# resibots/limbo

Measured on NVIDIA H100. Metric: GP fit+query/s at N=16384,D=6 (fit = K-build+Cholesky+alpha, query = 10k UCB candidates+argmax, fp64), higher is better.
Workload: dtype f64

## Files before the change

limbo_b200/csrc/gemm.cuh:

```cuda
#pragma once
#include "common.cuh"

namespace lbg {

constexpr int BM = 128;
constexpr int STAGES = 3;
constexpr int MMA_K = 4;

template <int BN_, int WN_, int BK_>
struct Cfg {
    static constexpr int BN = BN_, WN = WN_, BK = BK_;
    static constexpr int THREADS = 128 * WN;
    static constexpr int NT = BN / (8 * WN);
    static constexpr int PITCH_A_OC = BM + 4;
    static constexpr int PITCH_B_OC = BN + 4;
    static constexpr int PITCH_KC = BK + 4;
    static constexpr int A_STAGE = (BM * PITCH_KC > BK * PITCH_A_OC) ? BM * PITCH_KC : BK * PITCH_A_OC;
    static constexpr int B_STAGE = (BN * PITCH_KC > BK * PITCH_B_OC) ? BN * PITCH_KC : BK * PITCH_B_OC;
    static constexpr size_t PIPE_BYTES = (size_t)STAGES * (A_STAGE + B_STAGE) * sizeof(double);
    static constexpr int A_PIPE_DOUBLES = STAGES * A_STAGE;
    static_assert(BN % (8 * WN) == 0 && BK % MMA_K == 0, "tile shape");
    static_assert(PITCH_KC % 16 == 4 && PITCH_A_OC % 16 == 4 && PITCH_B_OC % 16 == 4, "conflict-free pitches");
};
using CfgWide = Cfg<128, 4, 32>;
using CfgDual = Cfg<64, 2, 16>;
using CfgStep = Cfg<64, 4, 32>;

template <typename C, bool KC, int NOUTER, int PITCH_OC>
struct TilePlan {
    static constexpr int CHUNKS = NOUTER * C::BK / 2;
    static constexpr int PER_THREAD = (CHUNKS + C::THREADS - 1) / C::THREADS;
    static constexpr int CPR = KC ? C::BK / 2 : NOUTER / 2;
    static constexpr int ROWS_PER_Q = C::THREADS / CPR;
    static constexpr int SSTEP = ROWS_PER_Q * (KC ? C::PITCH_KC : PITCH_OC);
    static_assert(C::THREADS % CPR == 0, "every chunk of a thread sits in the same column of the slab");
    int64_t goff, gstep;
    int soff;
    __device__ __forceinline__ void init(int64_t ld)
    {
        const int row = threadIdx.x / CPR, cc = threadIdx.x - row * CPR;
        goff = (int64_t)row * ld + 2 * cc;
        gstep = (int64_t)ROWS_PER_Q * ld;
        soff = row * (KC ? C::PITCH_KC : PITCH_OC) + 2 * cc;
    }
    __device__ __forceinline__ void issue(double* s, const double* __restrict__ g) const
    {
        s += soff;
        g += goff;
#pragma unroll
        for (int q = 0; q < PER_THREAD; ++q)
            if (CHUNKS % C::THREADS == 0 || (int)threadIdx.x + q * C::THREADS < CHUNKS) lb_cp_async16(s + q * SSTEP, g + q * gstep);
    }
};

template <typename C>
struct Acc {
    double v[2][C::NT][4];
    __device__ __forceinline__ void zero()
    {
#pragma unroll
        for (int a = 0; a < 2; ++a)
#pragma unroll
            for (int b = 0; b < C::NT; ++b)
#pragma unroll
                for (int c = 0; c < 4; ++c) v[a][b][c] = 0.0;
    }
};

template <typename C, bool NEG_A, typename FA, typename FB>
__device__ __forceinline__ void mma_kstep(Acc<C>& acc, FA fa, FB fb)
{
    double a[2][MMA_K / 2], b[C::NT][MMA_K / 4];
#pragma unroll
    for (int mt = 0; mt < 2; ++mt)
#pragma unroll
        for (int i = 0; i < MMA_K / 2; ++i) {
            a[mt][i] = fa(mt * 16 + 8 * (i & 1), 4 * (i >> 1));
            if (NEG_A) a[mt][i] = -a[mt][i];
        }
#pragma unroll
    for (int nt = 0; nt < C::NT; ++nt)
#pragma unroll
        for (int i = 0; i < MMA_K / 4; ++i) b[nt][i] = fb(nt * 8, 4 * i);
#pragma unroll
    for (int nt = 0; nt < C::NT; ++nt)
#pragma unroll
        for (int mt = 0; mt < 2; ++mt) lb_dmma_16x8<MMA_K>(acc.v[mt][nt], a[mt], b[nt]);
}

template <typename C, bool A_KC, bool B_KC, bool NEG_A>
__device__ __forceinline__ void compute_stage(Acc<C>& acc, const double* sA, const double* sB)
{
    const int lane = threadIdx.x & 31, warp = threadIdx.x >> 5;
    const int g = lane >> 2, t = lane & 3;
    const int wm = warp & 3, wn = warp >> 2;
    const int m_base = wm * 32 + g, n_base = wn * (C::BN / C::WN) + g;
#pragma unroll 2
    for (int k0 = 0; k0 < C::BK; k0 += MMA_K) {
        const int k = k0 + t;
        mma_kstep<C, NEG_A>(
            acc,
            [&](int dm, int dk) { return A_KC ? sA[(m_base + dm) * C::PITCH_KC + k + dk] : sA[(k + dk) * C::PITCH_A_OC + m_base + dm]; },
            [&](int dn, int dk) { return B_KC ? sB[(n_base + dn) * C::PITCH_KC + k + dk] : sB[(k + dk) * C::PITCH_B_OC + n_base + dn]; });
    }
}

template <typename C, bool A_KC, bool B_KC, bool NEG_A = false>
__device__ __forceinline__ void mainloop(Acc<C>& acc, const double* __restrict__ gA, int64_t lda,
    const double* __restrict__ gB, int64_t ldb, int K, double* smem)
{
    double* sA = smem;
    double* sB = smem + C::A_PIPE_DOUBLES;
    const int nk = K / C::BK;
    const int64_t stepA = A_KC ? C::BK : (int64_t)C::BK * lda;
    const int64_t stepB = B_KC ? C::BK : (int64_t)C::BK * ldb;
    TilePlan<C, A_KC, BM, C::PITCH_A_OC> pa;
    TilePlan<C, B_KC, C::BN, C::PITCH_B_OC> pb;
    pa.init(lda);
    pb.init(ldb);
#pragma unroll
    for (int s = 0; s < STAGES - 1; ++s) {
        if (s < nk) {
            pa.issue(sA + s * C::A_STAGE, gA + s * stepA);
            pb.issue(sB + s * C::B_STAGE, gB + s * stepB);
        }
        lb_cp_async_commit();
    }
    for (int kt = 0; kt < nk; ++kt) {
        lb_cp_async_wait<STAGES - 2>();
        __syncthreads();
        const int s = kt % STAGES;
        compute_stage<C, A_KC, B_KC, NEG_A>(acc, sA + s * C::A_STAGE, sB + s * C::B_STAGE);
        const int nx = kt + STAGES - 1;
        if (nx < nk) {
            const int sn = nx % STAGES;
            pa.issue(sA + sn * C::A_STAGE, gA + nx * stepA);
            pb.issue(sB + sn * C::B_STAGE, gB + nx * stepB);
        }
        lb_cp_async_commit();
    }
    lb_cp_async_wait<0>();
    __syncthreads();
}

template <typename C, typename F>
__device__ __forceinline__ void for_each_acc(Acc<C>& acc, F&& f)
{
    const int lane = threadIdx.x & 31, warp = threadIdx.x >> 5;
    const int g = lane >> 2, t = lane & 3;
    const int wm = warp & 3, wn = warp >> 2;
#pragma unroll
    for (int mt = 0; mt < 2; ++mt)
#pragma unroll
        for (int nt = 0; nt < C::NT; ++nt)
#pragma unroll
            for (int i = 0; i < 4; ++i) {
                int row = wm * 32 + mt * 16 + g + 8 * (i >> 1);
                int col = wn * (C::BN / C::WN) + nt * 8 + 2 * t + (i & 1);
                f(row, col, acc.v[mt][nt][i]);
            }
}

template <typename C>
__device__ __forceinline__ void load_acc(Acc<C>& acc, const double* __restrict__ Cg, int64_t ld)
{
    for_each_acc<C>(acc, [&](int r, int c, double& v) { v = __ldcs(Cg + r + (int64_t)c * ld); });
}
template <typename C>
__device__ __forceinline__ void store_acc(Acc<C>& acc, double* __restrict__ Cg, int64_t ld)
{
    for_each_acc<C>(acc, [&](int r, int c, double& v) { Cg[r + (int64_t)c * ld] = v; });
}

template <typename C>
__device__ __forceinline__ void mainloop_resB(Acc<C>& acc, const double* __restrict__ gA, int64_t lda,
    const double* sBres, double* smem_pipe)
{
    constexpr int PB = BM + 4;
    constexpr int nk = BM / C::BK;
    const int lane = threadIdx.x & 31, warp = threadIdx.x >> 5;
    const int g = lane >> 2, t = lane & 3;
    const int wm = warp & 3, wn = warp >> 2;
    const int m_base = wm * 32 + g, n_base = wn * (C::BN / C::WN) + g;
    TilePlan<C, false, BM, C::PITCH_A_OC> pa;
    pa.init(lda);
#pragma unroll
    for (int s = 0; s < STAGES - 1; ++s) {
        pa.issue(smem_pipe + s * C::A_STAGE, gA + (int64_t)s * C::BK * lda);
        lb_cp_async_commit();
    }
    for (int kt = 0; kt < nk; ++kt) {
        lb_cp_async_wait<STAGES - 2>();
        __syncthreads();
        const int nx = kt + STAGES - 1;
        if (nx < nk) pa.issue(smem_pipe + (nx % STAGES) * C::A_STAGE, gA + (int64_t)nx * C::BK * lda);
        lb_cp_async_commit();
        const double* sA = smem_pipe + (kt % STAGES) * C::A_STAGE;
#pragma unroll
        for (int k0 = 0; k0 < C::BK; k0 += MMA_K) {
            const int k = k0 + t;
            mma_kstep<C, false>(
                acc, [&](int dm, int dk) { return sA[(k + dk) * C::PITCH_A_OC + m_base + dm]; },
                [&](int dn, int dk) { return sBres[(n_base + dn) * PB + kt * C::BK + k + dk]; });
        }
    }
    lb_cp_async_wait<0>();
    __syncthreads();
}

}
```

limbo_b200/csrc/potrf.cu:

```cuda
#include "gemm.cuh"
#include <cstdlib>

namespace {

constexpr int PS = LB_TILE + 4;
constexpr int XP = 36;
constexpr int XB = 32 * XP;
constexpr size_t POTF2_SMEM = (size_t)(LB_TILE * PS + 10 * XB + LB_TILE) * sizeof(double);

__device__ __forceinline__ int blk(int ib, int jb) { return ib * (ib + 1) / 2 + jb; }

template <typename FA, typename FB>
__device__ __forceinline__ void warp_mma(double (&c)[4], int K, FA fa, FB fb)
{
    constexpr int KS = lbg::MMA_K;
    const int lane = threadIdx.x & 31, g = lane >> 2, t = lane & 3;
    for (int k0 = 0; k0 < K; k0 += KS) {
        double a[KS / 2], b[KS / 4];
#pragma unroll
        for (int i = 0; i < KS / 2; ++i) a[i] = fa(g + 8 * (i & 1), k0 + t + 4 * (i >> 1));
#pragma unroll
        for (int i = 0; i < KS / 4; ++i) b[i] = fb(k0 + t + 4 * i, g);
        lb_dmma_16x8<KS>(c, a, b);
    }
// ... 138 lines not shown
        }
        __syncthreads();
        const double* Xd = Xb + blk(ib, ib) * XB;
        for (int w = warp; w < 8 * ib; w += 8) {
            const int jb = w >> 3, mt = (w >> 2) & 1, nt = w & 3;
            double c[4] = {0.0, 0.0, 0.0, 0.0};
            warp_mma(c, 32, [&](int m, int kk) { return Xd[kk * XP + 16 * mt + m]; },
                [&](int kk, int n) { return S[(32 * ib + 8 * nt + n) * PS + 32 * jb + kk]; });
            double* Xo = Xb + blk(ib, jb) * XB;
#pragma unroll
            for (int e = 0; e < 4; ++e) Xo[(8 * nt + 2 * t + (e & 1)) * XP + 16 * mt + g + 8 * (e >> 1)] = -c[e];
        }
        __syncthreads();
    }
    LB_TICK();
    double* inv_out = invD + (int64_t)k * LB_TILE * LB_TILE;
    for (int idx = tid; idx < LB_TILE * (LB_TILE / 2); idx += 256) {
        const int c = idx >> 6, r = (idx & 63) * 2;
        if (c > r + 1) continue;
        if (do_factor) {
            double2 v = *reinterpret_cast<const double2*>(&S[c * PS + r]);
            if (c > r) v.x = 0.0;
            if (c > r + 1) v.y = 0.0;
            *reinterpret_cast<double2*>(Lkk + r + (int64_t)c * ld) = v;
        }
        double2 x = make_double2(0.0, 0.0);
        if (c <= r + 1) {
            const double* Xs_ = Xb + blk(r >> 5, c >> 5) * XB + (c & 31) * XP + (r & 31);
            x = *reinterpret_cast<const double2*>(Xs_);
            if (c > r) x.x = 0.0;
        }
        *reinterpret_cast<double2*>(inv_out + r + c * LB_TILE) = x;
    }
    __syncthreads();
    LB_TICK();
#undef LB_TICK
}

__global__ void __launch_bounds__(lbg::CfgWide::THREADS, 1)
trsm_panel_kernel(double* __restrict__ L, int64_t ld, int k, const double* __restrict__ invD)
{
    using C = lbg::CfgWide;
    extern __shared__ __align__(16) double smem[];
    const int i = k + 1 + blockIdx.x;
    double* A = L + (int64_t)i * LB_TILE + (int64_t)k * LB_TILE * ld;
    const double* B = invD + (int64_t)k * LB_TILE * LB_TILE;
    lbg::Acc<C> acc;
    acc.zero();
    lbg::mainloop<C, false, false>(acc, A, ld, B, LB_TILE, LB_TILE, smem);
    lbg::store_acc<C>(acc, A, ld);
}

template <typename C>
__global__ void __launch_bounds__(C::THREADS, (C::THREADS == 256) ? 2 : 1)
syrk_kernel(double* __restrict__ L, int64_t ld, int kb, int kd, int j0, int nc, int T)
{
    extern __shared__ __align__(16) double smem[];
    constexpr int SPLIT = LB_TILE / C::BN;
    int idx = blockIdx.x / SPLIT, c = 0;
    const int h = blockIdx.x - idx * SPLIT;
    while (c < nc && idx >= T - j0 - c) { idx -= T - j0 - c; ++c; }
    const int j = j0 + c, i = j + idx;
    const double* A = L + (int64_t)i * LB_TILE + (int64_t)kb * LB_TILE * ld;
    const double* B = L + (int64_t)j * LB_TILE + h * C::BN + (int64_t)kb * LB_TILE * ld;
    double* Cg = L + (int64_t)i * LB_TILE + ((int64_t)j * LB_TILE + h * C::BN) * ld;
    lbg::Acc<C> acc;
    lbg::load_acc<C>(acc, Cg, ld);
    lbg::mainloop<C, false, false, true>(acc, A, ld, B, ld, kd * LB_TILE, smem);
    lbg::store_acc<C>(acc, Cg, ld);
}

using SyrkCfg = lbg::CfgDual;
constexpr int SYRK_SPLIT = LB_TILE / SyrkCfg::BN;

LbOncePerDevice g_attr_once;
int set_attrs()
{
    if (!g_attr_once.need()) return LB_OK;
    LB_CUDA(cudaFuncSetAttribute(potf2_inv_kernel, cudaFuncAttributeMaxDynamicSharedMemorySize, (int)POTF2_SMEM));
    LB_CUDA(cudaFuncSetAttribute(trsm_panel_kernel, cudaFuncAttributeMaxDynamicSharedMemorySize, (int)lbg::CfgWide::PIPE_BYTES));
    LB_CUDA(cudaFuncSetAttribute(syrk_kernel<SyrkCfg>, cudaFuncAttributeMaxDynamicSharedMemorySize, (int)SyrkCfg::PIPE_BYTES));
    LB_CUDA(cudaFuncSetAttribute(syrk_kernel<lbg::CfgWide>, cudaFuncAttributeMaxDynamicSharedMemorySize, (int)lbg::CfgWide::PIPE_BYTES));
    return LB_OK;
}

}

int lb_debug_potf2_clocks(lb_gp* h, int k, long long* out_host, int n)
{
    int rc = set_attrs();
    if (rc) return rc;
    long long* d = nullptr;
    LB_CUDA(cudaMalloc(&d, sizeof(long long) * 16));
    LB_CUDA(cudaMemset(d, 0, sizeof(long long) * 16));
    potf2_inv_kernel<<<1, 256, POTF2_SMEM, h->stream>>>(h->dL, h->Np, k, h->dInvD, h->dInfo, 1, d);
    LB_CUDA(cudaStreamSynchronize(h->stream));
    LB_CUDA(cudaMemcpy(out_host, d, sizeof(long long) * (n < 16 ? n : 16), cudaMemcpyDeviceToHost));
    cudaFree(d);
    return LB_OK;
}

int lb_launch_potf2_block(lb_gp* h, int k, int do_factor)
{
    int rc = set_attrs();
    if (rc) return rc;
    potf2_inv_kernel<<<1, 256, POTF2_SMEM, h->stream>>>(h->dL, h->Np, k, h->dInvD, h->dInfo, do_factor);
    h->launches++;
    LB_CUDA(cudaGetLastError());
    return LB_OK;
}

static inline int syrk_tiles(int T, int j0, int nc)
{
    int n = 0;
    for (int c = 0; c < nc; ++c) n += T - j0 - c;
    return n;
}

static int launch_pair_panel(lb_gp* h, cudaStream_t side, int k, int T, int64_t ld)
{
    {
        LbProfScope ps(h, side, LB_PC_POTF2);
        potf2_inv_kernel<<<1, 256, POTF2_SMEM, side>>>(h->dL, ld, k, h->dInvD, h->dInfo, 1);
    }
    h->launches++;
    if (k + 1 < T) {
        {
            LbProfScope ps(h, side, LB_PC_TRSM_PANEL);
            trsm_panel_kernel<<<T - k - 1, lbg::CfgWide::THREADS, lbg::CfgWide::PIPE_BYTES, side>>>(h->dL, ld, k, h->dInvD);
        }
        {
            LbProfScope ps(h, side, LB_PC_SYRK_COL);
            syrk_kernel<SyrkCfg><<<(T - k - 1) * SYRK_SPLIT, SyrkCfg::THREADS, SyrkCfg::PIPE_BYTES, side>>>(h->dL, ld, k, 1, k + 1, 1, T);
        }
        {
            LbProfScope ps(h, side, LB_PC_POTF2);
            potf2_inv_kernel<<<1, 256, POTF2_SMEM, side>>>(h->dL, ld, k + 1, h->dInvD, h->dInfo, 1);
        }
        h->launches += 3;
        if (k + 2 < T) {
            LbProfScope ps(h, side, LB_PC_TRSM_PANEL);
            trsm_panel_kernel<<<T - k - 2, lbg::CfgWide::THREADS, lbg::CfgWide::PIPE_BYTES, side>>>(h->dL, ld, k + 1, h->dInvD);
            h->launches++;
        }
    }
    LB_CUDA(cudaGetLastError());
    return LB_OK;
}

static int launch_potrf_quads(lb_gp* h)
{
    const int T = (int)(h->Np / LB_TILE);
    const int64_t ld = h->Np;
    cudaStream_t main = h->stream, side = h->side ? h->side : h->stream;
    LB_CUDA(cudaMemsetAsync(h->dInfo, 0, 2 * sizeof(int), main));
    if (side != main) {
        LB_CUDA(cudaEventRecord(h->ev[0], main));
        LB_CUDA(cudaStreamWaitEvent(side, h->ev[0], 0));
    }
    int rc, q = 0;
    for (int k = 0; k < T; k += 4, ++q) {
        if ((rc = launch_pair_panel(h, side, k, T, ld))) return rc;
        if (k + 2 < T) {
            const int nc2 = (T - (k + 2) < 2) ? (T - (k + 2)) : 2;
            {
                LbProfScope ps(h, side, LB_PC_SYRK_COL);
                syrk_kernel<SyrkCfg><<<syrk_tiles(T, k + 2, nc2) * SYRK_SPLIT, SyrkCfg::THREADS, SyrkCfg::PIPE_BYTES, side>>>(h->dL, ld, k, 2, k + 2, nc2, T);
            }
            h->launches++;
            if ((rc = launch_pair_panel(h, side, k + 2, T, ld))) return rc;
        }
        if (k + 4 >= T) break;
        if (side != main) {
            LB_CUDA(cudaEventRecord(h->ev[1 + (q & 1)], side));
            LB_CUDA(cudaStreamWaitEvent(main, h->ev[1 + (q & 1)], 0));
        }
        const int j0 = k + 4;
        const int nca = (T - j0 < 4) ? (T - j0) : 4;
        static int wide = -1;
        if (wide < 0) { const char* e = getenv("LB_SYRK_WIDE"); wide = (e && atoi(e) != 0) ? 1 : 0; }
        {
            LbProfScope ps(h, main, LB_PC_SYRK);
            syrk_kernel<SyrkCfg><<<syrk_tiles(T, j0, nca) * SYRK_SPLIT, SyrkCfg::THREADS, SyrkCfg::PIPE_BYTES, main>>>(h->dL, ld, k, 4, j0, nca, T);
        }
        h->launches++;
        if (side != main) {
            LB_CUDA(cudaEventRecord(h->ev[3 + (q & 1)], main));
            LB_CUDA(cudaStreamWaitEvent(side, h->ev[3 + (q & 1)], 0));
        }
        const int ncb = T - j0 - nca;
        if (ncb > 0) {
            LbProfScope ps(h, main, LB_PC_SYRK);
            if (wide)
                syrk_kernel<lbg::CfgWide><<<syrk_tiles(T, j0 + nca, ncb), lbg::CfgWide::THREADS, lbg::CfgWide::PIPE_BYTES, main>>>(h->dL, ld, k, 4, j0 + nca,
                    ncb, T);
            else
                syrk_kernel<SyrkCfg><<<syrk_tiles(T, j0 + nca, ncb) * SYRK_SPLIT, SyrkCfg::THREADS, SyrkCfg::PIPE_BYTES, main>>>(h->dL, ld, k, 4, j0 + nca, ncb, T);
            h->launches++;
        }
    }
    if (side != main) {
        LB_CUDA(cudaEventRecord(h->ev[5], side));
        LB_CUDA(cudaStreamWaitEvent(main, h->ev[5], 0));
    }
    LB_CUDA(cudaGetLastError());
    return LB_OK;
}

int lb_launch_potrf(lb_gp* h)
{
    int rc = set_attrs();
    if (rc) return rc;
    static int quad = -1;
    if (quad < 0) { const char* e = getenv("LB_POTRF_QUAD"); quad = (e && atoi(e) == 0) ? 0 : 1; }
    if (quad) return launch_potrf_quads(h);
    const int T = (int)(h->Np / LB_TILE);
    const int64_t ld = h->Np;
    cudaStream_t main = h->stream, side = h->side ? h->side : h->stream;
    static int split_on = -1;
    if (split_on < 0) { const char* e = getenv("LB_POTRF_SPLIT"); split_on = (e && atoi(e) != 0) ? 1 : 0; }
    cudaStream_t second = main;
    if (split_on && T >= 24 && side != main) {
        if (!h->aux && cudaStreamCreateWithFlags(&h->aux, cudaStreamNonBlocking) != cudaSuccess) h->aux = nullptr;
        if (h->aux) second = h->aux;
    }
    const int cstar = (second != main) ? (((int)(0.38 * T)) & ~1) : T;
    LB_CUDA(cudaMemsetAsync(h->dInfo, 0, 2 * sizeof(int), main));
    if (side != main) {
        LB_CUDA(cudaEventRecord(h->ev[0], main));
        LB_CUDA(cudaStreamWaitEvent(side, h->ev[0], 0));
        if (second != main) LB_CUDA(cudaStreamWaitEvent(second, h->ev[0], 0));
    }
    int p = 0;
    for (int k = 0; k < T; k += 2, ++p) {
        const bool pair = (k + 1 < T);
        {
            LbProfScope ps(h, side, LB_PC_POTF2);
            potf2_inv_kernel<<<1, 256, POTF2_SMEM, side>>>(h->dL, ld, k, h->dInvD, h->dInfo, 1);
        }
        h->launches++;
        if (pair) {
            {
                LbProfScope ps(h, side, LB_PC_TRSM_PANEL);
                trsm_panel_kernel<<<T - k - 1, lbg::CfgWide::THREADS, lbg::CfgWide::PIPE_BYTES, side>>>(h->dL, ld, k, h->dInvD);
            }
            {
                LbProfScope ps(h, side, LB_PC_SYRK_COL);
                syrk_kernel<SyrkCfg><<<(T - k - 1) * SYRK_SPLIT, SyrkCfg::THREADS, SyrkCfg::PIPE_BYTES, side>>>(h->dL, ld, k, 1, k + 1, 1, T);
            }
            {
// ... 45 lines not shown
            if (ncb > 0) {
                LbProfScope ps(h, sa, LB_PC_SYRK);
                syrk_kernel<SyrkCfg><<<syrk_tiles(T, jb, ncb) * SYRK_SPLIT, SyrkCfg::THREADS, SyrkCfg::PIPE_BYTES, sa>>>(h->dL, ld, k, 2, jb, ncb, T);
                h->launches++;
            }
        }
    }
    if (side != main) {
        LB_CUDA(cudaEventRecord(h->ev[5], side));
        LB_CUDA(cudaStreamWaitEvent(main, h->ev[5], 0));
    }
    if (second != main) {
        LB_CUDA(cudaEventRecord(h->ev[6], second));
        LB_CUDA(cudaStreamWaitEvent(main, h->ev[6], 0));
    }
    LB_CUDA(cudaGetLastError());
    return LB_OK;
}

namespace {

__device__ __forceinline__ int dchol_global_block(int l, int rank, int G) { return 2 * (G * (l >> 1) + rank) + (l & 1); }

__global__ void __launch_bounds__(256)
dchol_build_kernel(const double* __restrict__ Xs, int64_t xs_ld, int64_t N, int64_t Nd, KernParams kp, int rank, int G, int64_t ncols_local,
    double* __restrict__ dLoc)
{
    const int64_t i = (int64_t)blockIdx.y * 256 + threadIdx.x;
    const int64_t c = blockIdx.x;
    if (i >= Nd || c >= ncols_local) return;
    const int64_t j = (int64_t)dchol_global_block((int)(c / LB_TILE), rank, G) * LB_TILE + (c % LB_TILE);
    double v;
    if (i >= N || j >= N) v = (i == j) ? 1.0 : 0.0;
    else {
        double z = 0.0;
        for (int d = 0; d < kp.D; ++d) {
            const double q = Xs[(int64_t)d * xs_ld + i] - Xs[(int64_t)d * xs_ld + j];
            z = fma(q, q, z);
        }
        v = lb_kernel_from_z(kp.id, z, kp) + ((i == j) ? kp.noise + 1e-8 : 0.0);
    }
    dLoc[i + c * Nd] = v;
}

__global__ void __launch_bounds__(256)
dchol_pack_kernel(const double* __restrict__ cols, int64_t ld, int64_t row0, double* __restrict__ panel, int64_t ldp)
{
    const int64_t r = (int64_t)blockIdx.x * 256 + threadIdx.x;
    const int c = blockIdx.y;
    if (r < ldp) panel[r + c * ldp] = cols[row0 + r + c * ld];
}

template <typename C>
__global__ void __launch_bounds__(C::THREADS, (C::THREADS == 256) ? 2 : 1)
dchol_update_kernel(double* __restrict__ Lloc, int64_t ld, const double* __restrict__ P, int64_t ldp, int kpair, int l0, int l1, int rank,
    int G, int T)
{
    extern __shared__ __align__(16) double smem[];
    constexpr int SPLIT = LB_TILE / C::BN;
    int idx = blockIdx.x / SPLIT;
    const int h = blockIdx.x - idx * SPLIT;
    int l = l0;
    for (; l < l1; ++l) {
        const int nt = T - dchol_global_block(l, rank, G);
        if (idx < nt) break;
        idx -= nt;
    }
    if (l >= l1) return;
    const int j = dchol_global_block(l, rank, G), i = j + idx;
    const int b0 = kpair + 2;
    const double* A = P + (int64_t)(i - b0) * LB_TILE;
    const double* B = P + (int64_t)(j - b0) * LB_TILE + h * C::BN;
    double* Cg = Lloc + (int64_t)i * LB_TILE + ((int64_t)l * LB_TILE + h * C::BN) * ld;
    lbg::Acc<C> acc;
    lbg::load_acc<C>(acc, Cg, ld);
    lbg::mainloop<C, false, false, true>(acc, A, ldp, B, ldp, 2 * LB_TILE, smem);
    lbg::store_acc<C>(acc, Cg, ld);
}

__global__ void __launch_bounds__(256)
dchol_finish_kernel(double* __restrict__ Lloc, int64_t ld, int64_t N, int rank, int G, int64_t ncols_local, double* __restrict__ part)
{
    __shared__ double red[8];
    double s = 0.0;
    for (int64_t c = blockIdx.x; c < ncols_local; c += gridDim.x) {
        const int64_t j = (int64_t)dchol_global_block((int)(c / LB_TILE), rank, G) * LB_TILE + (c % LB_TILE);
        double* col = Lloc + c * ld;
        for (int64_t i = threadIdx.x; i < j && i < ld; i += 256) col[i] = 0.0;
        if (threadIdx.x == 0 && j < N) s += log(col[j]);
    }
    s = lb_warp_sum(s);
    if ((threadIdx.x & 31) == 0) red[threadIdx.x >> 5] = s;
    __syncthreads();
    if (threadIdx.x == 0) {
        double t = 0.0;
        for (int w = 0; w < 8; ++w) t += red[w];
        part[blockIdx.x] = t;
    }
}
__global__ void dchol_sum_kernel(const double* __restrict__ part, int n, double* __restrict__ out)
{
    double s = 0.0;
    for (int i = 0; i < n; ++i) s += part[i];
    *out = s;
}

LbOncePerDevice g_dchol_once;
// ... 81 lines not shown
```

limbo_b200/csrc/query.cu:

```cuda
#include "gemm.cuh"
#include <cfloat>
#include <cstdlib>

namespace {

constexpr int DCH = 16;

__global__ void __launch_bounds__(256, 2)
kstar_kernel(const double* __restrict__ Xs, int64_t Np, int64_t N, const double* __restrict__ Qs, int64_t Mp,
    int64_t M, double* __restrict__ V, KernParams kp)
{
    __shared__ __align__(128) double sxi[DCH][LB_TILE];
    __shared__ __align__(128) double sxj[DCH][LB_TILE];
    __shared__ __align__(8) uint64_t bar;
    const int tid = threadIdx.x, lane = tid & 31, warp = tid >> 5;
    const int li = lane & 7, lj = lane >> 3;
    const int D = kp.D;
    const int64_t i0 = (int64_t)blockIdx.x * LB_TILE, j0 = (int64_t)blockIdx.y * LB_TILE;
    const int r0 = warp * 16 + 2 * li;
    if (tid == 0) {
        lb_mbar_init(&bar, 1);
        lb_fence_barrier_init();
    }
    __syncthreads();
// ... 590 lines not shown
        __syncthreads();
        if (tid < ncols && c0 + tid < M) {
            double res = kp.sf2 - sNrm[tid];
            res = (res <= DBL_EPSILON) ? 0.0 : res;
            s2_out[c0 + tid] = res + kp.noise;
            for (int p = 0; p < P; ++p) mu_out[(c0 + tid) * P + p] = sMu[p * SLAB + tid];
        }
        __syncthreads();
    }
}

__global__ void __launch_bounds__(THREADS, 1)
query_slab_kernel(const double* __restrict__ L, int64_t ld, const double* __restrict__ invD, const double* __restrict__ Xs,
    int64_t N, const double* __restrict__ Qs, int64_t Mp, int64_t M, const double* __restrict__ alpha, int P, KernParams kp,
    double* __restrict__ Vscratch, int nslabs, int64_t ntiles_total, double* __restrict__ mu_out, double* __restrict__ s2_out)
{
    extern __shared__ __align__(16) double sm[];
    double* V = Vscratch + (int64_t)blockIdx.x * ld * SLAB;
    for (int s = blockIdx.x; s < nslabs; s += gridDim.x) {
        const int64_t t0 = ntiles_total * s / nslabs, t1 = ntiles_total * (s + 1) / nslabs;
        const int ntc = (int)(t1 - t0);
        if (ntc == 9) slab_body<9>(sm, L, ld, invD, Xs, N, Qs, Mp, M, alpha, P, kp, V, t0, ntc, mu_out, s2_out);
        else if (ntc == 8) slab_body<8>(sm, L, ld, invD, Xs, N, Qs, Mp, M, alpha, P, kp, V, t0, ntc, mu_out, s2_out);
        else slab_body<0>(sm, L, ld, invD, Xs, N, Qs, Mp, M, alpha, P, kp, V, t0, ntc, mu_out, s2_out);
    }
}

struct PointArg { double x[LB_MAX_D]; };

__global__ void __launch_bounds__(THREADS, 1)
query_point_kernel(const double* __restrict__ L, int64_t ld, const double* __restrict__ invD, const double* __restrict__ Xs, int64_t N,
    const __grid_constant__ PointArg q, double* __restrict__ Qs, const double* __restrict__ alpha, int P, const __grid_constant__ KernParams kp,
    double* __restrict__ Vscratch, double* __restrict__ out)
{
    extern __shared__ __align__(16) double sm[];
    for (int idx = threadIdx.x; idx < kp.D * 8; idx += THREADS) {
        const int d = idx >> 3, c = idx & 7;
        Qs[d * LB_TILE + c] = (c == 0) ? lb_staged_coord(kp, d, [&](int r) { return q.x[r]; }) : 0.0;
    }
    __threadfence_block();
    __syncthreads();
    slab_body<0>(sm, L, ld, invD, Xs, N, Qs, LB_TILE, 1, alpha, P, kp, Vscratch, 0, 1, out, out + P);
}

LbOncePerDevice g_attr_once2;

}

namespace panel {

constexpr int SB = 16;

template <typename C, bool INV>
__global__ void __launch_bounds__(C::THREADS, (C::THREADS == 256) ? 2 : 1)
panel_update_kernel(const double* __restrict__ L, int64_t ld, const double* __restrict__ V, double* __restrict__ Tbuf, int64_t ldt, int s0,
    int nrows, int ct0, int inv_rank, int inv_G)
{
    extern __shared__ __align__(16) double smem[];
    const int i = blockIdx.x % nrows, ct = ct0 + blockIdx.x / nrows;
    int kb = 0;
    if (INV) {
        const int c = inv_rank + (ct * C::BN / LB_TILE) * inv_G;
        if (c >= s0 + nrows) return;
        kb = c / SB * SB;
    }
    const double* Vc = V + (int64_t)ct * C::BN * ld;
    lbg::Acc<C> acc;
    lbg::load_acc<C>(acc, Vc + (int64_t)(s0 + i) * LB_TILE, ld);
    if (s0 > kb)
        lbg::mainloop<C, false, true, true>(acc, L + (int64_t)(s0 + i) * LB_TILE + (int64_t)kb * LB_TILE * ld, ld, Vc + (int64_t)kb * LB_TILE, ld,
            (s0 - kb) * LB_TILE, smem);
    lbg::store_acc<C>(acc, Tbuf + (int64_t)i * LB_TILE + (int64_t)ct * C::BN * ldt, ldt);
}

template <typename C, bool INV>
__global__ void __launch_bounds__(C::THREADS, (C::THREADS == 256) ? 2 : 1)
panel_solve_kernel(const double* __restrict__ Linv, int64_t ld, const double* __restrict__ Tbuf, int64_t ldt, double* __restrict__ V, int s0,
    int nrows, double* __restrict__ normpart, int64_t Mp, int ct0, int inv_rank, int inv_G)
{
    extern __shared__ __align__(16) double smem[];
    const int i = nrows - 1 - (int)(blockIdx.x % nrows), ct = ct0 + blockIdx.x / nrows;
    int k0 = 0;
    if (INV) {
        const int c = inv_rank + (ct * C::BN / LB_TILE) * inv_G;
        if (c >= s0 + nrows) return;
        if (c > s0) k0 = c - s0;
        if (i < k0) return;
    }
    lbg::Acc<C> acc;
    acc.zero();
    lbg::mainloop<C, false, true>(acc, Linv + (int64_t)(s0 + i) * LB_TILE + (int64_t)(s0 + k0) * LB_TILE * ld, ld,
        Tbuf + (int64_t)k0 * LB_TILE + (int64_t)ct * C::BN * ldt, ldt, (i + 1 - k0) * LB_TILE, smem);
    lbg::store_acc<C>(acc, V + (int64_t)(s0 + i) * LB_TILE + (int64_t)ct * C::BN * ld, ld);
    if (INV) return;
    const int lane = threadIdx.x & 31, warp = threadIdx.x >> 5;
    const int g = lane >> 2, t = lane & 3;
    const int wm = warp & 3, wn = warp >> 2;
    double* sRed = smem;
#pragma unroll
    for (int nt = 0; nt < C::NT; ++nt)
#pragma unroll
        for (int e = 0; e < 2; ++e) {
            double sq = 0.0;
#pragma unroll
            for (int mt = 0; mt < 2; ++mt) {
                sq = fma(acc.v[mt][nt][e], acc.v[mt][nt][e], sq);
                sq = fma(acc.v[mt][nt][2 + e], acc.v[mt][nt][2 + e], sq);
            }
#pragma unroll
            for (int o = 4; o < 32; o <<= 1) sq += __shfl_xor_sync(0xffffffffu, sq, o);
            if (g == 0) sRed[wm * C::BN + wn * (C::BN / C::WN) + nt * 8 + 2 * t + e] = sq;
        }
    __syncthreads();
    if ((int)threadIdx.x < C::BN) {
        const double sum = ((sRed[threadIdx.x] + sRed[C::BN + threadIdx.x]) + sRed[2 * C::BN + threadIdx.x]) + sRed[3 * C::BN + threadIdx.x];
        normpart[(int64_t)(s0 + i) * Mp + (int64_t)ct * C::BN + threadIdx.x] = sum;
    }
}

__global__ void __launch_bounds__(256)
panel_finish_kernel(const double* __restrict__ normpart, int T, int64_t Mp, int64_t M, double kvv, double noise, double* __restrict__ s2)
{
    const int64_t c = blockIdx.x * (int64_t)256 + threadIdx.x;
    if (c >= M) return;
    double s = 0.0;
    for (int tt = 0; tt < T; ++tt) s += normpart[(int64_t)tt * Mp + c];
    double res = kvv - s;
    res = (res <= DBL_EPSILON) ? 0.0 : res;
    s2[c] = res + noise;
}

LbOncePerDevice g_once;

}

size_t lb_query_panel_scratch_doubles(const lb_gp* h, int64_t Mp)
{
    const int64_t T = h->Np / LB_TILE;
    return (size_t)(h->Np * Mp + (int64_t)panel::SB * LB_TILE * Mp + T * Mp);
}

int lb_launch_query_panel(lb_gp* h, cudaStream_t st, int64_t M, const double* dQs, int64_t Mp, double* dWork, double* dMu, double* dS2,
    long long* launches)
{
    using namespace panel;
    using CW = lbg::CfgWide;
    using CD = lbg::CfgDual;
    if (g_once.need()) {
        LB_CUDA(cudaFuncSetAttribute(panel_update_kernel<CW, false>, cudaFuncAttributeMaxDynamicSharedMemorySize, (int)CW::PIPE_BYTES));
        LB_CUDA(cudaFuncSetAttribute(panel_solve_kernel<CW, false>, cudaFuncAttributeMaxDynamicSharedMemorySize, (int)CW::PIPE_BYTES));
        LB_CUDA(cudaFuncSetAttribute(panel_update_kernel<CD, false>, cudaFuncAttributeMaxDynamicSharedMemorySize, (int)CD::PIPE_BYTES));
        LB_CUDA(cudaFuncSetAttribute(panel_solve_kernel<CD, false>, cudaFuncAttributeMaxDynamicSharedMemorySize, (int)CD::PIPE_BYTES));
    }
    const int T = (int)(h->Np / LB_TILE);
    const int64_t ld = h->Np, ldt = (int64_t)SB * LB_TILE;
    double* dV = dWork;
    double* dT = dV + ld * Mp;
    double* dNorm = dT + ldt * Mp;
    int rc = lb_launch_linv_levels(h, SB);
    if (rc) return rc;
    dim3 grid((unsigned)T, (unsigned)(Mp / LB_TILE));
    {
        LbProfScope ps(h, st, LB_PC_KSTAR);
        kstar_kernel<<<grid, 256, 0, st>>>(h->dXs, h->Np, h->N, dQs, Mp, M, dV, h->kp);
    }
    {
        LbProfScope ps(h, st, LB_PC_QREDUCE);
        mu_kernel<<<(unsigned)M, 256, 0, st>>>(dV, h->Np, h->dAlpha, h->P, dMu);
    }
    if (launches) *launches += 2;
    const int ctiles = (int)(Mp / LB_TILE);
    static int split_pct = -1, use_side = -1;
    if (split_pct < 0) {
        const char* e = getenv("LB_PANEL_SPLIT");
        split_pct = e ? atoi(e) : 100;
        if (split_pct < 1 || split_pct > 100) split_pct = 100;
        const char* e2 = getenv("LB_PANEL_SIDE");
        use_side = (e2 && atoi(e2) != 0) ? 1 : 0;
    }
    static int cfg_mode = -1;
    if (cfg_mode < 0) { const char* e = getenv("LB_PANEL_CFG"); cfg_mode = e ? atoi(e) : 0; }
    const bool dual = cfg_mode != 1;
    const int wmul = dual ? 2 : 1;
    static int force_groups = -1;
    if (force_groups < 0) { const char* e = getenv("LB_PANEL_GROUPS"); force_groups = e ? atoi(e) : 0; }
    int sms = 132;
    cudaDeviceGetAttribute(&sms, cudaDevAttrMultiProcessorCount, h->device);
    const int slots = sms * (dual ? 2 : 1);
    int ngroups = 1;
    if (ctiles >= 4 && (int64_t)ctiles * wmul * SB < (int64_t)slots) ngroups = 4;
    else if (split_pct < 100 && ctiles >= 4) ngroups = 2;
    if (force_groups >= 1 && force_groups <= 4) ngroups = force_groups;
    if (ngroups > ctiles) ngroups = ctiles;
    cudaStream_t sts[4] = {st, st, st, st};
    if (ngroups >= 2) {
        if (use_side && h->side && ngroups == 2) sts[1] = h->side;
        else {
            cudaStream_t* extra[3] = {&h->aux, &h->aux2, &h->aux3};
            for (int g = 1; g < ngroups; ++g) {
                if (!*extra[g - 1] && cudaStreamCreateWithFlags(extra[g - 1], cudaStreamNonBlocking) != cudaSuccess) *extra[g - 1] = nullptr;
                if (!*extra[g - 1]) { ngroups = g; break; }
                sts[g] = *extra[g - 1];
            }
        }
    }
    int gbeg[5] = {0, ctiles, ctiles, ctiles, ctiles};
    if (ngroups == 2) {
        int split = (ctiles * split_pct + 50) / 100;
        if (split < 1) split = 1;
        if (split > ctiles - 1) split = ctiles - 1;
        gbeg[1] = split;
    }
    else
        for (int g = 1; g < ngroups; ++g) gbeg[g] = (int)((int64_t)ctiles * g / ngroups);
    gbeg[ngroups] = ctiles;
    {
        LbProfScope ps(h, st, LB_PC_QSTEP);
        if (ngroups >= 2) {
            LB_CUDA(cudaEventRecord(h->ev[0], st));
            for (int g = 1; g < ngroups; ++g) LB_CUDA(cudaStreamWaitEvent(sts[g], h->ev[0], 0));
        }
        for (int s0 = 0; s0 < T; s0 += SB) {
            const int nrows = (T - s0 < SB) ? (T - s0) : SB;
            for (int g = 0; g < ngroups; ++g) {
                const int c0 = gbeg[g] * wmul, nc = (gbeg[g + 1] - gbeg[g]) * wmul;
                if (nc <= 0) continue;
                if (dual) {
                    panel_update_kernel<CD, false><<<nrows * nc, CD::THREADS, CD::PIPE_BYTES, sts[g]>>>(h->dL, ld, dV, dT, ldt, s0, nrows, c0, 0, 1);
                    panel_solve_kernel<CD, false><<<nrows * nc, CD::THREADS, CD::PIPE_BYTES, sts[g]>>>(h->dLinv, ld, dT, ldt, dV, s0, nrows, dNorm, Mp, c0, 0, 1);
                }
                else {
                    panel_update_kernel<CW, false><<<nrows * nc, CW::THREADS, CW::PIPE_BYTES, sts[g]>>>(h->dL, ld, dV, dT, ldt, s0, nrows, c0, 0, 1);
                    panel_solve_kernel<CW, false><<<nrows * nc, CW::THREADS, CW::PIPE_BYTES, sts[g]>>>(h->dLinv, ld, dT, ldt, dV, s0, nrows, dNorm, Mp, c0, 0, 1);
                }
                if (launches) *launches += 2;
            }
        }
        for (int g = 1; g < ngroups; ++g) {
            LB_CUDA(cudaEventRecord(h->ev[g], sts[g]));
            LB_CUDA(cudaStreamWaitEvent(st, h->ev[g], 0));
        }
    }
    {
        LbProfScope ps(h, st, LB_PC_QREDUCE);
        panel_finish_kernel<<<(unsigned)((M + 255) / 256), 256, 0, st>>>(dNorm, T, Mp, M, h->kp.sf2, h->kp.noise, dS2);
    }
    if (launches) ++*launches;
    LB_CUDA(cudaGetLastError());
    return LB_OK;
}

namespace panel {
__global__ void __launch_bounds__(128)
identity_cols_kernel(double* __restrict__ V, int64_t ld, int rank, int G, int T)
{
    const int c = rank + (int)blockIdx.x * G;
    if (c >= T) return;
    V[(int64_t)c * LB_TILE + threadIdx.x + ((int64_t)blockIdx.x * LB_TILE + threadIdx.x) * ld] = 1.0;
}
LbOncePerDevice g_once_inv;
}

int64_t lb_linv_columns_width(const lb_gp* h, int G) { return ((h->Np / LB_TILE + G - 1) / G) * LB_TILE; }

size_t lb_linv_columns_scratch_doubles(const lb_gp* h, int G)
{
    const int64_t Mp = lb_linv_columns_width(h, G);
    return (size_t)(h->Np * Mp + (int64_t)panel::SB * LB_TILE * Mp);
}

int lb_launch_linv_columns(lb_gp* h, cudaStream_t st, int rank, int G, double* dWork, long long* launches)
{
    using namespace panel;
    using CD = lbg::CfgDual;
    if (g_once_inv.need()) {
        LB_CUDA(cudaFuncSetAttribute(panel_update_kernel<CD, true>, cudaFuncAttributeMaxDynamicSharedMemorySize, (int)CD::PIPE_BYTES));
        LB_CUDA(cudaFuncSetAttribute(panel_solve_kernel<CD, true>, cudaFuncAttributeMaxDynamicSharedMemorySize, (int)CD::PIPE_BYTES));
    }
    const int T = (int)(h->Np / LB_TILE);
    const int nt = (T + G - 1) / G;
    const int64_t ld = h->Np, ldt = (int64_t)SB * LB_TILE, Mp = (int64_t)nt * LB_TILE;
    double* dV = dWork;
    double* dT = dV + ld * Mp;
    int rc = lb_launch_linv_levels(h, SB);
    if (rc) return rc;
    LbProfScope ps(h, st, LB_PC_TRTRI);
    LB_CUDA(cudaMemsetAsync(dV, 0, sizeof(double) * (size_t)(ld * Mp), st));
// ... 51 lines not shown
```

Before: 9.276.

## Reshape dual panel GEMM config to 2x2 warps with 64x32 warp tiles

Generalizes the GEMM Cfg with a configurable warp-row count and CTAs-per-SM, and switches the dual panel config from 4x2 warps (256 threads) to 2x2 warps (128 threads), so each warp computes a larger 64x32 tile. Launch bounds now come from the config, and the panel-solve norm epilogue is rewritten to reduce over multiple 32-row slices per warp before the shared-memory sum. Larger warp tiles improve register-level reuse of A/B fragments but raise register pressure and halve threads per CTA, which may hurt latency hiding. The unused wide syrk and panel code paths and their env switches are removed.

```diff
diff --git a/limbo_b200/csrc/gemm.cuh b/limbo_b200/csrc/gemm.cuh
--- a/limbo_b200/csrc/gemm.cuh
+++ b/limbo_b200/csrc/gemm.cuh
@@ -7,11 +7,14 @@
 constexpr int STAGES = 3;
 constexpr int MMA_K = 4;
 
-template <int BN_, int WN_, int BK_>
+template <int BN_, int WN_, int BK_, int WM_ = 4, int CTAS_ = 1>
 struct Cfg {
-    static constexpr int BN = BN_, WN = WN_, BK = BK_;
-    static constexpr int THREADS = 128 * WN;
+    static constexpr int BN = BN_, WN = WN_, BK = BK_, WM = WM_;
+    static constexpr int CTAS_PER_SM = CTAS_;
+    static constexpr int THREADS = 32 * WM * WN;
+    static constexpr int MT = BM / (16 * WM);
     static constexpr int NT = BN / (8 * WN);
+    static constexpr int WTM = 16 * MT, WTN = 8 * NT;
     static constexpr int PITCH_A_OC = BM + 4;
     static constexpr int PITCH_B_OC = BN + 4;
     static constexpr int PITCH_KC = BK + 4;
@@ -19,11 +22,11 @@
     static constexpr int B_STAGE = (BN * PITCH_KC > BK * PITCH_B_OC) ? BN * PITCH_KC : BK * PITCH_B_OC;
     static constexpr size_t PIPE_BYTES = (size_t)STAGES * (A_STAGE + B_STAGE) * sizeof(double);
     static constexpr int A_PIPE_DOUBLES = STAGES * A_STAGE;
-    static_assert(BN % (8 * WN) == 0 && BK % MMA_K == 0, "tile shape");
+    static_assert(BN % (8 * WN) == 0 && BM % (32 * WM) == 0 && (WM & (WM - 1)) == 0 && BK % MMA_K == 0, "tile shape");
     static_assert(PITCH_KC % 16 == 4 && PITCH_A_OC % 16 == 4 && PITCH_B_OC % 16 == 4, "conflict-free pitches");
 };
 using CfgWide = Cfg<128, 4, 32>;
-using CfgDual = Cfg<64, 2, 16>;
+using CfgDual = Cfg<64, 2, 16, 2, 2>;
 using CfgStep = Cfg<64, 4, 32>;
 
 template <typename C, bool KC, int NOUTER, int PITCH_OC>
@@ -55,24 +58,29 @@
 
 template <typename C>
 struct Acc {
-    double v[2][C::NT][4];
+    double v[C::MT][C::NT][4];
     __device__ __forceinline__ void zero()
     {
 #pragma unroll
-        for (int a = 0; a < 2; ++a)
+        for (int a = 0; a < C::MT; ++a)
 #pragma unroll
             for (int b = 0; b < C::NT; ++b)
 #pragma unroll
                 for (int c = 0; c < 4; ++c) v[a][b][c] = 0.0;
     }
 };
+
+template <typename C>
+__device__ __forceinline__ int warp_row0() { return ((int)(threadIdx.x >> 5) & (C::WM - 1)) * C::WTM; }
+template <typename C>
+__device__ __forceinline__ int warp_col0() { return ((int)(threadIdx.x >> 5) / C::WM) * C::WTN; }
 
 template <typename C, bool NEG_A, typename FA, typename FB>
 __device__ __forceinline__ void mma_kstep(Acc<C>& acc, FA fa, FB fb)
 {
-    double a[2][MMA_K / 2], b[C::NT][MMA_K / 4];
-#pragma unroll
-    for (int mt = 0; mt < 2; ++mt)
+    double a[C::MT][MMA_K / 2], b[C::NT][MMA_K / 4];
+#pragma unroll
+    for (int mt = 0; mt < C::MT; ++mt)
 #pragma unroll
         for (int i = 0; i < MMA_K / 2; ++i) {
             a[mt][i] = fa(mt * 16 + 8 * (i & 1), 4 * (i >> 1));
@@ -85,16 +93,15 @@
 #pragma unroll
     for (int nt = 0; nt < C::NT; ++nt)
 #pragma unroll
-        for (int mt = 0; mt < 2; ++mt) lb_dmma_16x8<MMA_K>(acc.v[mt][nt], a[mt], b[nt]);
+        for (int mt = 0; mt < C::MT; ++mt) lb_dmma_16x8<MMA_K>(acc.v[mt][nt], a[mt], b[nt]);
 }
 
 template <typename C, bool A_KC, bool B_KC, bool NEG_A>
 __device__ __forceinline__ void compute_stage(Acc<C>& acc, const double* sA, const double* sB)
 {
-    const int lane = threadIdx.x & 31, warp = threadIdx.x >> 5;
+    const int lane = threadIdx.x & 31;
     const int g = lane >> 2, t = lane & 3;
-    const int wm = warp & 3, wn = warp >> 2;
-    const int m_base = wm * 32 + g, n_base = wn * (C::BN / C::WN) + g;
+    const int m_base = warp_row0<C>() + g, n_base = warp_col0<C>() + g;
 #pragma unroll 2
     for (int k0 = 0; k0 < C::BK; k0 += MMA_K) {
         const int k = k0 + t;
@@ -146,17 +153,17 @@
 template <typename C, typename F>
 __device__ __forceinline__ void for_each_acc(Acc<C>& acc, F&& f)
 {
-    const int lane = threadIdx.x & 31, warp = threadIdx.x >> 5;
+    const int lane = threadIdx.x & 31;
     const int g = lane >> 2, t = lane & 3;
-    const int wm = warp & 3, wn = warp >> 2;
-#pragma unroll
-    for (int mt = 0; mt < 2; ++mt)
+    const int row0 = warp_row0<C>(), col0 = warp_col0<C>();
+#pragma unroll
+    for (int mt = 0; mt < C::MT; ++mt)
 #pragma unroll
         for (int nt = 0; nt < C::NT; ++nt)
 #pragma unroll
             for (int i = 0; i < 4; ++i) {
-                int row = wm * 32 + mt * 16 + g + 8 * (i >> 1);
-                int col = wn * (C::BN / C::WN) + nt * 8 + 2 * t + (i & 1);
+                int row = row0 + mt * 16 + g + 8 * (i >> 1);
+                int col = col0 + nt * 8 + 2 * t + (i & 1);
                 f(row, col, acc.v[mt][nt][i]);
             }
 }
@@ -178,10 +185,9 @@
 {
     constexpr int PB = BM + 4;
     constexpr int nk = BM / C::BK;
-    const int lane = threadIdx.x & 31, warp = threadIdx.x >> 5;
+    const int lane = threadIdx.x & 31;
     const int g = lane >> 2, t = lane & 3;
-    const int wm = warp & 3, wn = warp >> 2;
-    const int m_base = wm * 32 + g, n_base = wn * (C::BN / C::WN) + g;
+    const int m_base = warp_row0<C>() + g, n_base = warp_col0<C>() + g;
     TilePlan<C, false, BM, C::PITCH_A_OC> pa;
     pa.init(lda);
 #pragma unroll
diff --git a/limbo_b200/csrc/potrf.cu b/limbo_b200/csrc/potrf.cu
--- a/limbo_b200/csrc/potrf.cu
+++ b/limbo_b200/csrc/potrf.cu
@@ -214,7 +214,7 @@
 }
 
 template <typename C>
-__global__ void __launch_bounds__(C::THREADS, (C::THREADS == 256) ? 2 : 1)
+__global__ void __launch_bounds__(C::THREADS, C::CTAS_PER_SM)
 syrk_kernel(double* __restrict__ L, int64_t ld, int kb, int kd, int j0, int nc, int T)
 {
     extern __shared__ __align__(16) double smem[];
@@ -242,7 +242,6 @@
     LB_CUDA(cudaFuncSetAttribute(potf2_inv_kernel, cudaFuncAttributeMaxDynamicSharedMemorySize, (int)POTF2_SMEM));
     LB_CUDA(cudaFuncSetAttribute(trsm_panel_kernel, cudaFuncAttributeMaxDynamicSharedMemorySize, (int)lbg::CfgWide::PIPE_BYTES));
     LB_CUDA(cudaFuncSetAttribute(syrk_kernel<SyrkCfg>, cudaFuncAttributeMaxDynamicSharedMemorySize, (int)SyrkCfg::PIPE_BYTES));
-    LB_CUDA(cudaFuncSetAttribute(syrk_kernel<lbg::CfgWide>, cudaFuncAttributeMaxDynamicSharedMemorySize, (int)lbg::CfgWide::PIPE_BYTES));
     return LB_OK;
 }
 
@@ -339,8 +338,6 @@
         }
         const int j0 = k + 4;
         const int nca = (T - j0 < 4) ? (T - j0) : 4;
-        static int wide = -1;
-        if (wide < 0) { const char* e = getenv("LB_SYRK_WIDE"); wide = (e && atoi(e) != 0) ? 1 : 0; }
         {
             LbProfScope ps(h, main, LB_PC_SYRK);
             syrk_kernel<SyrkCfg><<<syrk_tiles(T, j0, nca) * SYRK_SPLIT, SyrkCfg::THREADS, SyrkCfg::PIPE_BYTES, main>>>(h->dL, ld, k, 4, j0, nca, T);
@@ -353,11 +350,7 @@
         const int ncb = T - j0 - nca;
         if (ncb > 0) {
             LbProfScope ps(h, main, LB_PC_SYRK);
-            if (wide)
-                syrk_kernel<lbg::CfgWide><<<syrk_tiles(T, j0 + nca, ncb), lbg::CfgWide::THREADS, lbg::CfgWide::PIPE_BYTES, main>>>(h->dL, ld, k, 4, j0 + nca,
-                    ncb, T);
-            else
-                syrk_kernel<SyrkCfg><<<syrk_tiles(T, j0 + nca, ncb) * SYRK_SPLIT, SyrkCfg::THREADS, SyrkCfg::PIPE_BYTES, main>>>(h->dL, ld, k, 4, j0 + nca, ncb, T);
+            syrk_kernel<SyrkCfg><<<syrk_tiles(T, j0 + nca, ncb) * SYRK_SPLIT, SyrkCfg::THREADS, SyrkCfg::PIPE_BYTES, main>>>(h->dL, ld, k, 4, j0 + nca, ncb, T);
             h->launches++;
         }
     }
@@ -509,7 +502,7 @@
 }
 
 template <typename C>
-__global__ void __launch_bounds__(C::THREADS, (C::THREADS == 256) ? 2 : 1)
+__global__ void __launch_bounds__(C::THREADS, C::CTAS_PER_SM)
 dchol_update_kernel(double* __restrict__ Lloc, int64_t ld, const double* __restrict__ P, int64_t ldp, int kpair, int l0, int l1, int rank,
     int G, int T)
 {
diff --git a/limbo_b200/csrc/query.cu b/limbo_b200/csrc/query.cu
--- a/limbo_b200/csrc/query.cu
+++ b/limbo_b200/csrc/query.cu
@@ -666,7 +666,7 @@
 constexpr int SB = 16;
 
 template <typename C, bool INV>
-__global__ void __launch_bounds__(C::THREADS, (C::THREADS == 256) ? 2 : 1)
+__global__ void __launch_bounds__(C::THREADS, C::CTAS_PER_SM)
 panel_update_kernel(const double* __restrict__ L, int64_t ld, const double* __restrict__ V, double* __restrict__ Tbuf, int64_t ldt, int s0,
     int nrows, int ct0, int inv_rank, int inv_G)
 {
@@ -688,7 +688,7 @@
 }
 
 template <typename C, bool INV>
-__global__ void __launch_bounds__(C::THREADS, (C::THREADS == 256) ? 2 : 1)
+__global__ void __launch_bounds__(C::THREADS, C::CTAS_PER_SM)
 panel_solve_kernel(const double* __restrict__ Linv, int64_t ld, const double* __restrict__ Tbuf, int64_t ldt, double* __restrict__ V, int s0,
     int nrows, double* __restrict__ normpart, int64_t Mp, int ct0, int inv_rank, int inv_G)
 {
@@ -705,26 +705,33 @@
     acc.zero();
     lbg::mainloop<C, false, true>(acc, Linv + (int64_t)(s0 + i) * LB_TILE + (int64_t)(s0 + k0) * LB_TILE * ld, ld,
         Tbuf + (int64_t)k0 * LB_TILE + (int64_t)ct * C::BN * ldt, ldt, (i + 1 - k0) * LB_TILE, smem);
+    if (INV) {
+        lbg::store_acc<C>(acc, V + (int64_t)(s0 + i) * LB_TILE + (int64_t)ct * C::BN * ld, ld);
+        return;
+    }
+    constexpr int SL = C::MT / 2;
+    static_assert(C::MT % 2 == 0 && C::THREADS >= C::BN, "norm epilogue: whole 32-row slices per warp, a thread per column");
+    const int lane = threadIdx.x & 31;
+    const int g = lane >> 2, t = lane & 3;
+    const int slice0 = lbg::warp_row0<C>() / 32, col0 = lbg::warp_col0<C>();
+    double* sRed = smem;
+#pragma unroll
+    for (int sl = 0; sl < SL; ++sl)
+#pragma unroll
+        for (int nt = 0; nt < C::NT; ++nt)
+#pragma unroll
+            for (int e = 0; e < 2; ++e) {
+                double sq = 0.0;
+#pragma unroll
+                for (int mt = 2 * sl; mt < 2 * sl + 2; ++mt) {
+                    sq = fma(acc.v[mt][nt][e], acc.v[mt][nt][e], sq);
+                    sq = fma(acc.v[mt][nt][2 + e], acc.v[mt][nt][2 + e], sq);
+                }
+#pragma unroll
+                for (int o = 4; o < 32; o <<= 1) sq += __shfl_xor_sync(0xffffffffu, sq, o);
+                if (g == 0) sRed[(slice0 + sl) * C::BN + col0 + nt * 8 + 2 * t + e] = sq;
+            }
     lbg::store_acc<C>(acc, V + (int64_t)(s0 + i) * LB_TILE + (int64_t)ct * C::BN * ld, ld);
-    if (INV) return;
-    const int lane = threadIdx.x & 31, warp = threadIdx.x >> 5;
-    const int g = lane >> 2, t = lane & 3;
-    const int wm = warp & 3, wn = warp >> 2;
-    double* sRed = smem;
-#pragma unroll
-    for (int nt = 0; nt < C::NT; ++nt)
-#pragma unroll
-        for (int e = 0; e < 2; ++e) {
-            double sq = 0.0;
-#pragma unroll
-            for (int mt = 0; mt < 2; ++mt) {
-                sq = fma(acc.v[mt][nt][e], acc.v[mt][nt][e], sq);
-                sq = fma(acc.v[mt][nt][2 + e], acc.v[mt][nt][2 + e], sq);
-            }
-#pragma unroll
-            for (int o = 4; o < 32; o <<= 1) sq += __shfl_xor_sync(0xffffffffu, sq, o);
-            if (g == 0) sRed[wm * C::BN + wn * (C::BN / C::WN) + nt * 8 + 2 * t + e] = sq;
-        }
     __syncthreads();
     if ((int)threadIdx.x < C::BN) {
         const double sum = ((sRed[threadIdx.x] + sRed[C::BN + threadIdx.x]) + sRed[2 * C::BN + threadIdx.x]) + sRed[3 * C::BN + threadIdx.x];
@@ -758,11 +765,8 @@
     long long* launches)
 {
     using namespace panel;
-    using CW = lbg::CfgWide;
     using CD = lbg::CfgDual;
     if (g_once.need()) {
-        LB_CUDA(cudaFuncSetAttribute(panel_update_kernel<CW, false>, cudaFuncAttributeMaxDynamicSharedMemorySize, (int)CW::PIPE_BYTES));
-        LB_CUDA(cudaFuncSetAttribute(panel_solve_kernel<CW, false>, cudaFuncAttributeMaxDynamicSharedMemorySize, (int)CW::PIPE_BYTES));
         LB_CUDA(cudaFuncSetAttribute(panel_update_kernel<CD, false>, cudaFuncAttributeMaxDynamicSharedMemorySize, (int)CD::PIPE_BYTES));
         LB_CUDA(cudaFuncSetAttribute(panel_solve_kernel<CD, false>, cudaFuncAttributeMaxDynamicSharedMemorySize, (int)CD::PIPE_BYTES));
     }
@@ -792,15 +796,12 @@
         const char* e2 = getenv("LB_PANEL_SIDE");
         use_side = (e2 && atoi(e2) != 0) ? 1 : 0;
     }
-    static int cfg_mode = -1;
-    if (cfg_mode < 0) { const char* e = getenv("LB_PANEL_CFG"); cfg_mode = e ? atoi(e) : 0; }
-    const bool dual = cfg_mode != 1;
-    const int wmul = dual ? 2 : 1;
+    constexpr int wmul = LB_TILE / CD::BN;
     static int force_groups = -1;
     if (force_groups < 0) { const char* e = getenv("LB_PANEL_GROUPS"); force_groups = e ? atoi(e) : 0; }
     int sms = 132;
     cudaDeviceGetAttribute(&sms, cudaDevAttrMultiProcessorCount, h->device);
-    const int slots = sms * (dual ? 2 : 1);
+    const int slots = sms * CD::CTAS_PER_SM;
     int ngroups = 1;
     if (ctiles >= 4 && (int64_t)ctiles * wmul * SB < (int64_t)slots) ngroups = 4;
     else if (split_pct < 100 && ctiles >= 4) ngroups = 2;
@@ -839,14 +840,8 @@
             for (int g = 0; g < ngroups; ++g) {
                 const int c0 = gbeg[g] * wmul, nc = (gbeg[g + 1] - gbeg[g]) * wmul;
                 if (nc <= 0) continue;
-                if (dual) {
-                    panel_update_kernel<CD, false><<<nrows * nc, CD::THREADS, CD::PIPE_BYTES, sts[g]>>>(h->dL, ld, dV, dT, ldt, s0, nrows, c0, 0, 1);
-                    panel_solve_kernel<CD, false><<<nrows * nc, CD::THREADS, CD::PIPE_BYTES, sts[g]>>>(h->dLinv, ld, dT, ldt, dV, s0, nrows, dNorm, Mp, c0, 0, 1);
-                }
-                else {
-                    panel_update_kernel<CW, false><<<nrows * nc, CW::THREADS, CW::PIPE_BYTES, sts[g]>>>(h->dL, ld, dV, dT, ldt, s0, nrows, c0, 0, 1);
-                    panel_solve_kernel<CW, false><<<nrows * nc, CW::THREADS, CW::PIPE_BYTES, sts[g]>>>(h->dLinv, ld, dT, ldt, dV, s0, nrows, dNorm, Mp, c0, 0, 1);
-                }
+                panel_update_kernel<CD, false><<<nrows * nc, CD::THREADS, CD::PIPE_BYTES, sts[g]>>>(h->dL, ld, dV, dT, ldt, s0, nrows, c0, 0, 1);
+                panel_solve_kernel<CD, false><<<nrows * nc, CD::THREADS, CD::PIPE_BYTES, sts[g]>>>(h->dLinv, ld, dT, ldt, dV, s0, nrows, dNorm, Mp, c0, 0, 1);
                 if (launches) *launches += 2;
             }
         }
```

After: 9.706 (median of 6 runs). 1.05x the previous value.
